# Chaos-Ray-Tracing-Vladislav/course-assignment-DanielHalachev

Measured on AMD Instinct MI355X. Metric: Mpixels/s at 1920x1080 depth 8; HBM GB/s vs roofline, higher is better.
Workload: dtype f32; 1 GPU; HW14 Optimizations02-like BVH scene: room + seeded torus knot + reflective and refractive spheres, four lights, 207954 triangles, 1920x1080, depth 8, 8x8 tiles dealt round-robin over 1 GPU(s); scene=hw14, width=1920, height=1080, max_depth=8, parallelism=tiles8x8-roundrobin-1, tuning=defaults

## Files before the change

course-assignment-danielhalachev_amd/csrc/crt_abi.hip:

```cpp
#include "crt_internal.h"

namespace {


__global__ void unpack_kernel(const float *packed, uint32_t n_parts, uint64_t part_stride, float *frame, uint32_t width,
                              uint32_t height, uint32_t tiles_x, uint32_t n_tiles) {
    const uint64_t gid = (uint64_t)blockIdx.x * blockDim.x + threadIdx.x;
    if (gid >= (uint64_t)n_tiles * 64) return;
    const uint32_t tile = (uint32_t)(gid >> 6), sub = (uint32_t)(gid & 63);
    const uint32_t px = (tile % tiles_x) * TILE + (sub & 7u), py = (tile / tiles_x) * TILE + (sub >> 3);
    if (px >= width || py >= height) return;
    const uint32_t part = tile % n_parts, local = tile / n_parts;
    const float *src = packed + (uint64_t)part * part_stride + ((uint64_t)local * 64 + sub) * 3;
    float *dst = frame + ((uint64_t)py * width + px) * 3;
    dst[0] = src[0]; dst[1] = src[1]; dst[2] = src[2];
}

__global__ void unpack_items_kernel(const float *packed, const WorkItem *items, uint32_t n_items, float *frame, uint32_t width,
                                    uint32_t height, uint32_t tiles_x) {
    const uint64_t gid = (uint64_t)blockIdx.x * blockDim.x + threadIdx.x;
    if (gid >= (uint64_t)n_items * 64) return;
    const WorkItem wi = items[gid >> 6];
    const uint32_t sub = (uint32_t)(gid & 63);
    const uint32_t px = (wi.tile % tiles_x) * TILE + (sub & 7u), py = (wi.tile / tiles_x) * TILE + (sub >> 3);
// ... 147 lines not shown
    const uint32_t n = crt_packed_tile_count(ctx, first, stride);
    crt_rect key{first, stride, 0u, 0u};
    bool same = ctx->cached_is_partition && ctx->cached_rects.size() == 1 && memcmp(ctx->cached_rects.data(), &key, sizeof(key)) == 0;
    if (!same) {
        std::vector<WorkItem> items(n);
        uint64_t pixels = 0;
        for (uint32_t j = 0; j < n; j++) {
            const uint32_t t = first + j * stride;
            const uint32_t tx = t % ctx->tiles_x, ty = t / ctx->tiles_x;
            const uint32_t w = (tx + 1) * TILE <= ctx->width ? TILE : ctx->width - tx * TILE;
            const uint32_t h = (ty + 1) * TILE <= ctx->height ? TILE : ctx->height - ty * TILE;
            pixels += (uint64_t)w * h;
            items[j] = WorkItem{t, j, ~0ull};
        }
        rc = ensure_items(ctx, n ? n : 1);
        if (rc) return rc;
        if (n) CRT_HIP_CHECK(ctx, hipMemcpy(ctx->d_items, items.data(), n * sizeof(WorkItem), hipMemcpyHostToDevice));
        ctx->cached_rects.assign(1, key);
        ctx->cached_is_partition = true;
        ctx->cached_n_items = n;
        ctx->cached_pixels = pixels;
    }
    rc = launch_render(ctx, o, n, d_packed, 1, (hipStream_t)stream);
    if (rc) return rc;
    if (o->collect_counters) {
        CRT_HIP_CHECK(ctx, hipStreamSynchronize((hipStream_t)stream));
        return fetch_counters(ctx, o, ctx->cached_pixels);
    }
    ctx->stats.pixels = ctx->cached_pixels;
    ctx->stats.counters_valid = 0;
    return CRT_OK;
}

extern "C" int crt_unpack_tiles_device(crt_ctx *ctx, const float *d_packed_all, uint32_t n_parts, uint64_t part_stride_floats,
                                       float *d_frame, void *stream) {
    if (!ctx || !d_packed_all || !d_frame || n_parts == 0) return CRT_ERR_INVALID;
    CRT_HIP_CHECK(ctx, hipSetDevice(ctx->device));
    const uint32_t n_tiles = ctx->tiles_x * ctx->tiles_y;
    const uint64_t tiles_per_part = ((uint64_t)n_tiles + n_parts - 1) / n_parts;
    if (part_stride_floats < tiles_per_part * 64 * 3) {
        ctx->error = "crt_unpack_tiles_device: part_stride_floats is smaller than one part's tiles (ceil(tiles / n_parts) * 192 floats)";
        return CRT_ERR_INVALID;
    }
    const uint64_t threads = (uint64_t)n_tiles * 64;
    hipLaunchKernelGGL(unpack_kernel, dim3((uint32_t)((threads + 255) / 256)), dim3(256), 0, (hipStream_t)stream, d_packed_all,
                       n_parts, part_stride_floats, d_frame, ctx->width, ctx->height, ctx->tiles_x, n_tiles);
    CRT_HIP_CHECK(ctx, hipGetLastError());
    return CRT_OK;
}

extern "C" int crt_quantize_device(crt_ctx *ctx, const float *d_rgb, uint64_t n_values, uint8_t *d_out, void *stream) {
    if (!ctx || !d_rgb || !d_out) return CRT_ERR_INVALID;
    CRT_HIP_CHECK(ctx, hipSetDevice(ctx->device));
    if (n_values == 0) return CRT_OK;
    hipLaunchKernelGGL(quantize_kernel, dim3((uint32_t)((n_values + 255) / 256)), dim3(256), 0, (hipStream_t)stream, d_rgb,
                       n_values, d_out);
    CRT_HIP_CHECK(ctx, hipGetLastError());
    return CRT_OK;
}

extern "C" int crt_read_quantized(crt_ctx *ctx, uint8_t *out_rgb8) {
    if (!ctx || !out_rgb8) return CRT_ERR_INVALID;
    const uint64_t n = (uint64_t)ctx->width * ctx->height * 3;
    int rc = crt_quantize_device(ctx, ctx->d_frame, n, ctx->d_quant, ctx->stream);
    if (rc) return rc;
    CRT_HIP_CHECK(ctx, hipMemcpyAsync(out_rgb8, ctx->d_quant, n, hipMemcpyDeviceToHost, ctx->stream));
    CRT_HIP_CHECK(ctx, hipStreamSynchronize(ctx->stream));
    return CRT_OK;
}

extern "C" int crt_kernel_elapsed_ms(crt_ctx *ctx, double *ms) {
    if (!ctx || !ms) return CRT_ERR_INVALID;
    CRT_HIP_CHECK(ctx, hipSetDevice(ctx->device));
    if (ctx->launches == 0) { ctx->error = "no render kernel has been launched"; return CRT_ERR_INVALID; }
    const int slot = (int)((ctx->launches - 1) % crt_ctx::EV_RING);
    CRT_HIP_CHECK(ctx, hipEventSynchronize(ctx->ev4[slot]));
    float f = 0;
    CRT_HIP_CHECK(ctx, hipEventElapsedTime(&f, ctx->ev0[slot], ctx->ev4[slot]));
    *ms = f;
    ctx->stats.kernel_ms = f;
    return CRT_OK;
}

extern "C" int crt_kernel_times_ms(crt_ctx *ctx, double *out_phase_ms, uint32_t max_count, uint32_t *count) {
    if (!ctx || !count) return CRT_ERR_INVALID;
    CRT_HIP_CHECK(ctx, hipSetDevice(ctx->device));
    uint64_t n = ctx->launches < (uint64_t)crt_ctx::EV_RING ? ctx->launches : (uint64_t)crt_ctx::EV_RING;
    if (n > max_count) n = max_count;
    for (uint64_t i = 0; i < n; i++) {
        const int slot = (int)((ctx->launches - n + i) % crt_ctx::EV_RING);
        CRT_HIP_CHECK(ctx, hipEventSynchronize(ctx->ev4[slot]));
        float t = 0, a = 0, b = 0, c = 0, e = 0;
        CRT_HIP_CHECK(ctx, hipEventElapsedTime(&t, ctx->ev0[slot], ctx->ev4[slot]));
        CRT_HIP_CHECK(ctx, hipEventElapsedTime(&a, ctx->ev0[slot], ctx->ev1[slot]));
        CRT_HIP_CHECK(ctx, hipEventElapsedTime(&b, ctx->ev_s0[slot], ctx->ev_s1[slot]));
        hipEvent_t e2 = ctx->ev2[slot];
        if (ctx->slot_ev2_is_s1[slot]) {
            CRT_HIP_CHECK(ctx, hipEventElapsedTime(&c, ctx->ev1[slot], ctx->ev_s1[slot]));
            e2 = c < 0.0f ? ctx->ev1[slot] : ctx->ev_s1[slot];
        }
        CRT_HIP_CHECK(ctx, hipEventElapsedTime(&c, ctx->ev1[slot], e2));
        CRT_HIP_CHECK(ctx, hipEventElapsedTime(&e, e2, ctx->ev3[slot]));
        if (out_phase_ms) {
            out_phase_ms[5 * i] = t; out_phase_ms[5 * i + 1] = a; out_phase_ms[5 * i + 2] = b;
            out_phase_ms[5 * i + 3] = c; out_phase_ms[5 * i + 4] = e;
        }
    }
    *count = (uint32_t)n;
    note_overflow(ctx);
    return CRT_OK;
}

extern "C" int crt_get_kernel_counters(crt_ctx *ctx, uint64_t closest[9], uint64_t shadow[9]) {
    if (!ctx || !closest || !shadow) return CRT_ERR_INVALID;
    for (int k = 0; k < C_PUBLIC; k++) { closest[k] = ctx->level_counters[k]; shadow[k] = ctx->shadow0_counters[k]; }
    return CRT_OK;
}

extern "C" int crt_get_executed_counters(crt_ctx *ctx, uint64_t out[4]) {
    if (!ctx || !out) return CRT_ERR_INVALID;
    out[0] = ctx->exec_counters[0] + ctx->exec_counters[2];
    out[1] = ctx->exec_counters[1] + ctx->exec_counters[3];
    out[2] = ctx->exec_counters[2];
    out[3] = ctx->exec_counters[3];
    return CRT_OK;
}

extern "C" int crt_get_executed_plan_tests(crt_ctx *ctx, uint64_t out[2]) {
    if (!ctx || !out) return CRT_ERR_INVALID;
    out[0] = ctx->exec_counters[4] + ctx->exec_counters[5];
    out[1] = ctx->exec_counters[5];
    return CRT_OK;
}

extern "C" int crt_debug_stream_counts(crt_ctx *ctx, uint32_t *out, uint32_t max_words) {
    if (!ctx || !out) return CRT_ERR_INVALID;
    CRT_HIP_CHECK(ctx, hipSetDevice(ctx->device));
    CRT_HIP_CHECK(ctx, hipDeviceSynchronize());
    const uint32_t n = max_words < (uint32_t)SC_ALLOC_WORDS ? max_words : (uint32_t)SC_ALLOC_WORDS;
    CRT_HIP_CHECK(ctx, hipMemcpy(out, ctx->d_scounts, n * sizeof(uint32_t), hipMemcpyDeviceToHost));
    return CRT_OK;
}

extern "C" int crt_describe_kernels(const crt_ctx *ctx, char *out, size_t size) {
    if (!ctx || !out || size == 0) return CRT_ERR_INVALID;
    const SceneArgs &A = ctx->scene;
    std::string d;
    if (ctx->mode == crt_ctx::MODE_LANES) d = "all=render_lanes<false>";
    else {
        const bool heavy = ctx->step_budget && A.nested_boxes && (A.top_fast || A.plan_seq);
        const bool lean = heavy && ctx->lean_ok && (A.plan_ok || A.plan_wide);
        const bool wide = lean && !A.plan_ok;
        const bool bvh = A.bvh_ok && ctx->tuning.bvh;
        if (bvh && ctx->tuning.level_queue) d = "level0=bvh_trace_level0<0>;shadow0=bvh_trace_shadow<0u, 0>;levels=bvh_trace_queue<0>";
        else if (bvh) d = "level0=bvh_trace_shade;shadow0=bvh_trace_shadow<0u, 0>;levels=bvh_trace_shade";
        else d = std::string("level0=") + (!lean ? "stream_trace_shade<false>" : wide ? "stream_trace_shade_plan_wide" : "stream_trace_shade_plan");
        if (!bvh) d += std::string(";shadow0=") + (!lean ? "stream_trace_shadow<false>" : wide ? "stream_trace_shadow_plan_wide<0u>" : "stream_trace_shadow_plan<0u>");
        if (!bvh) d += std::string(";levels=") + (!heavy ? "stream_trace_shade<false>" : "heavy_trace_closest");
    }
    d += std::string(";filter=") + (A.bvh_ok ? ctx->bvh_stats : "none (" + ctx->bvh_note + ")");
    snprintf(out, size, "%s", d.c_str());
    return CRT_OK;
}

extern "C" int crt_get_stats(crt_ctx *ctx, crt_stats *out) {
    if (!ctx || !out) return CRT_ERR_INVALID;
    *out = ctx->stats;
    return CRT_OK;
}

extern "C" int crt_synchronize(crt_ctx *ctx) {
    if (!ctx) return CRT_ERR_INVALID;
    CRT_HIP_CHECK(ctx, hipSetDevice(ctx->device));
    CRT_HIP_CHECK(ctx, hipDeviceSynchronize());
    note_overflow(ctx);
    return CRT_OK;
}
```

course-assignment-danielhalachev_amd/csrc/crt_internal.h:

```cpp
#pragma once

#include <hip/hip_runtime.h>

#include <algorithm>
#include <cfloat>
#include <cmath>
#include <cstdio>
#include <cstdlib>
#include <chrono>
#include <cstring>
#include <new>
#include <condition_variable>
#include <mutex>
#include <string>
#include <thread>
#include <vector>

#include "../../include/crt_hip.h"
#include "crt_bvh.h"
#include "kernel_common.h"

#define CRT_INTERNAL __attribute__((visibility("hidden")))

constexpr uint64_t QUERY_LAUNCH_RAYS = 1ull << 27;
constexpr uint64_t QUERY_HOST_RAYS = 1ull << 22;
constexpr uint64_t SHOOT_PASS_RAYS = 1ull << 22;

struct crt_ctx {
    int device = 0;
    std::string error;
    hipStream_t stream = nullptr;
    static constexpr int EV_RING = 64;
    hipEvent_t ev0[EV_RING] = {}, ev1[EV_RING] = {}, ev2[EV_RING] = {}, ev3[EV_RING] = {}, ev4[EV_RING] = {};
    hipEvent_t ev_fork[EV_RING] = {}, ev_s0[EV_RING] = {}, ev_s1[EV_RING] = {}, ev_s2[EV_RING] = {};
    bool slot_ev2_is_s1[EV_RING] = {};
    uint64_t launches = 0;
    uint32_t width = 0, height = 0, tiles_x = 0, tiles_y = 0;
    SceneArgs scene{};
    FrameArgs frame{};
    SceneArgs *d_scene = nullptr;
    FrameArgs *d_frame_ring = nullptr, *h_frame_ring = nullptr;
    const FrameArgs *h_frame_ring_dev = nullptr;
    std::vector<void *> allocs;
    float *d_frame = nullptr;
    uint8_t *d_quant = nullptr;
    WorkItem *d_items = nullptr;
    size_t items_cap = 0;
    std::vector<crt_rect> cached_rects;
    bool cached_is_partition = false;
    uint32_t cached_n_items = 0;
    uint64_t cached_pixels = 0;
    uint32_t *d_sync = nullptr;
    uint64_t level_counters[C_N] = {}, shadow0_counters[C_N] = {};
    enum Mode { MODE_STREAM, MODE_LANES } mode = MODE_STREAM;
    float4 *d_rayq[2] = {nullptr, nullptr};
    float4 *d_shadowq = nullptr;
    uint8_t *d_occluded = nullptr;
    float *d_kfac = nullptr;
    float4 *d_nodes = nullptr;
    uint32_t *d_scounts = nullptr;
    unsigned long long *d_exec = nullptr;
    unsigned long long exec_counters[6] = {0, 0, 0, 0, 0, 0};
    uint32_t *d_fallback_total = nullptr;
    uint32_t *d_heavy = nullptr;
    uint32_t *d_sheavy = nullptr;
    float4 *d_hits = nullptr;
    float4 *d_hits_all = nullptr;
    unsigned long long *d_lq = nullptr;
    uint32_t *d_lq_words = nullptr;
    uint32_t *d_bvh_spill = nullptr;
    uint32_t bvh_stack_built = 0;
    size_t bvh_spill_words() const { return bvh_stack_built > BVH_LDS_STACK ? (size_t)grid_blocks * BLOCK * (bvh_stack_built - BVH_LDS_STACK) : 0u; }
    hipStream_t side = nullptr;
    hipStream_t early = nullptr;
    hipEvent_t ev_reset[EV_RING] = {}, ev_queue[EV_RING] = {};
    static constexpr uint32_t H_SLOT_WORDS = 512;
    uint32_t *h_ring = nullptr;
    uint64_t next_count_harvest = 0;
    uint32_t slot_items[EV_RING] = {};
    std::vector<uint32_t> last_counts;
    uint32_t last_counts_items = 0;
    uint32_t fallbacks_seen = 0;
    double node_mult = 4.0, ray_mult = 2.0, shadow_extra = 1.0;
    uint32_t sizing_seen_fallbacks = 0;
    uint64_t queue_bytes = 0;
    uint64_t regrows = 0;
    uint32_t last_counts_cfg = 0;
    uint32_t slot_cfg[64] = {};
    hipEvent_t ev_call0 = nullptr, ev_call1 = nullptr;
    bool pending = false;
    crt_options pending_options{};
    uint32_t heavy_cap = 0;
    uint32_t step_budget = 384;
    bool lean_ok = true;
    uint64_t stream_items = 0;
    uint64_t overflows = 0;
    uint32_t n_lights = 0;
    crt_tuning tuning{};
    std::string bvh_note;
    std::string bvh_stats;
    unsigned long long *d_counters = nullptr;
    float *d_frames = nullptr;
    size_t frames_floats = 0;
    uint32_t grid_blocks = 0;
    crt_stats stats{};
    int num_cus = 0;
    struct crt_query_state *query = nullptr;
    uint64_t query_host_rays = QUERY_HOST_RAYS, query_launch_rays = QUERY_LAUNCH_RAYS, shoot_pass_rays = SHOOT_PASS_RAYS;
};

static constexpr uint32_t HEAVY_BLOCKS = 4096;
static constexpr uint32_t REFILL_BUNDLE = 16;

extern CRT_INTERNAL std::string g_create_error;

#define CRT_HIP_CHECK(ctx, expr)                                                                    \
    do {                                                                                            \
        hipError_t e_ = (expr);                                                                     \
        if (e_ != hipSuccess) {                                                                     \
            (ctx)->error = std::string(#expr) + ": " + hipGetErrorString(e_);                       \
            return CRT_ERR_HIP;                                                                     \
        }                                                                                           \
    } while (0)

template <typename T>
static int upload(crt_ctx *ctx, const T *src, size_t count, const T **dst) {
    void *p = nullptr;
    size_t bytes = (count ? count : 1) * sizeof(T);
    CRT_HIP_CHECK(ctx, hipMalloc(&p, bytes));
    ctx->allocs.push_back(p);
    if (count) CRT_HIP_CHECK(ctx, hipMemcpy(p, src, count * sizeof(T), hipMemcpyHostToDevice));
    *dst = (const T *)p;
    return CRT_OK;
}

CRT_INTERNAL int check_options(crt_ctx *ctx, const crt_options *o);
CRT_INTERNAL int ensure_items(crt_ctx *ctx, size_t n);
CRT_INTERNAL int launch_render(crt_ctx *ctx, const crt_options *o, uint32_t n_items, float *d_out, uint32_t packed, hipStream_t stream);
CRT_INTERNAL void note_overflow(crt_ctx *ctx);
CRT_INTERNAL int fetch_counters(crt_ctx *ctx, const crt_options *o, uint64_t pixels);
CRT_INTERNAL void query_destroy(crt_ctx *ctx);
CRT_INTERNAL uint64_t coverage_items(uint32_t width, uint32_t height, const crt_rect *rects, uint32_t n_rects, std::vector<WorkItem> &items);
CRT_INTERNAL void launch_unpack_items(const float *packed, const WorkItem *items, uint32_t n_items, float *frame, uint32_t width, uint32_t height,
                                      uint32_t tiles_x, hipStream_t stream);
```

course-assignment-danielhalachev_amd/csrc/crt_launch.hip:

```cpp
#include "crt_internal.h"
#include "glibc_powf.h"

namespace {

#include "kernel_lane.h"
#include "kernel_stream.h"
#include "kernel_heavy.h"
#include "kernel_plan.h"
#include "kernel_bvh.h"

}

int check_options(crt_ctx *ctx, const crt_options *o) {
    if (!o) { ctx->error = "options is NULL"; return CRT_ERR_INVALID; }
    if (o->use_gi && o->collect_counters == 2) { ctx->error = "collect_counters == 2 belongs to the ray-stream kernels; the GI mode renders with render_lanes"; return CRT_ERR_INVALID; }
    if (o->use_gi && (o->gi_sample_size > 64u || o->rays_per_pixel > 65536u)) { ctx->error = "gi_sample_size > 64 or rays_per_pixel > 65536"; return CRT_ERR_INVALID; }
    if (o->max_depth > 4096) { ctx->error = "max_depth too large"; return CRT_ERR_INVALID; }
    return CRT_OK;
}

int ensure_items(crt_ctx *ctx, size_t n) {
    if (n <= ctx->items_cap) return CRT_OK;
    CRT_HIP_CHECK(ctx, hipDeviceSynchronize());
    if (ctx->d_items) (void)hipFree(ctx->d_items);
// ... 134 lines not shown
        CRT_HIP_CHECK(ctx, hipMalloc((void **)&ctx->d_hits, (size_t)ctx->heavy_cap * sizeof(float4)));
        CRT_HIP_CHECK(ctx, hipMalloc((void **)&ctx->d_hits_all, (size_t)std::max<uint64_t>(ray_cap, px) * sizeof(float4)));
        if (ctx->scene.bvh_ok && ctx->tuning.bvh && ctx->tuning.level_queue) {
            CRT_HIP_CHECK(ctx, hipMalloc((void **)&ctx->d_lq, node_cap * 8 * sizeof(unsigned long long)));
            CRT_HIP_CHECK(ctx, hipMemset(ctx->d_lq, 0, node_cap * 8 * sizeof(unsigned long long)));
        }
        A.s_ray_cap = (uint32_t)ray_cap; A.s_shadow_cap = (uint32_t)shadow_cap; A.s_node_cap = (uint32_t)node_cap;
        ctx->stream_items = n_items;
        ctx->queue_bytes = ray_cap * 64 + shadow_cap * 37 + node_cap * 32 + (size_t)ctx->heavy_cap * 24 + std::max<uint64_t>(ray_cap, px) * 16 + (ctx->d_lq ? node_cap * 64 : 0);
    }
    A.s_rayq[0] = ctx->d_rayq[0]; A.s_rayq[1] = ctx->d_rayq[1];
    A.s_shadowq = ctx->d_shadowq; A.s_occluded = ctx->d_occluded; A.s_kfac = ctx->d_kfac; A.s_nodes = ctx->d_nodes;
    A.s_heavy = ctx->d_heavy; A.s_sheavy = ctx->d_sheavy; A.s_hits = ctx->d_hits; A.s_hits_all = ctx->d_hits_all; A.s_heavy_cap = ctx->heavy_cap;
    A.s_lq = ctx->d_lq; A.s_lq_cap = ctx->d_lq ? (ctx->tuning.ray_cap ? std::min(A.s_ray_cap, A.s_node_cap) : A.s_node_cap) : 0u;
    return CRT_OK;
}

static uint32_t level0_samples_of(const crt_options *o) { return o->use_gi && o->rays_per_pixel > 1u ? o->rays_per_pixel : 1u; }
static bool gi_fits_stream(const crt_options *o, uint32_t n_items) {
    return (uint64_t)n_items * 64u * level0_samples_of(o) * 2u < (1ull << 31) && o->gi_sample_size <= 64u;
}
static uint32_t frame_config_of(const crt_options *o) {
    return (o->use_gi ? 0x80000000u : 0u) | ((o->use_gi ? o->gi_sample_size & 0x7Fu : 0u) << 24) | (o->max_depth & 0xFFFFFFu);
}

static int g_debug_sync = 0;
template <typename K, typename... Args>
static void launch(K kernel, uint32_t blocks, hipStream_t stream, Args... args) {
    static int serial = 0;
    if (g_debug_sync) { fprintf(stderr, "[launch %d] kernel %p blocks %u ...", serial, (void *)kernel, blocks); fflush(stderr); }
    hipLaunchKernelGGL(kernel, dim3(blocks), dim3(BLOCK), 0, stream, args...);
    if (g_debug_sync) { hipError_t e = hipDeviceSynchronize(); fprintf(stderr, " done (%s)\n", hipGetErrorString(e)); fflush(stderr); serial++; }
}
template <typename K, typename... Args>
static void launch_lds(K kernel, uint32_t blocks, uint32_t lds_bytes, hipStream_t stream, Args... args) {
    hipLaunchKernelGGL(kernel, dim3(blocks), dim3(BLOCK), lds_bytes, stream, args...);
}

struct FramePlan {
    int slot;
    uint32_t n_items, vitems;
    uint32_t lane_blocks;
    bool gi, count, exec_count;
    bool heavy, lean, wide;
    bool bvh;
    bool queue;
    uint32_t widest;
    uint32_t level_budget;
    const uint32_t *prev;
    bool last_resort;
    bool one_stream;
};

static void launch_frame_reset(crt_ctx *ctx, const FramePlan &P, hipStream_t stream, bool stream_pass, uint32_t shadow_preset, uint32_t split_preset) {
    hipLaunchKernelGGL(stream_frame_reset, dim3(1), dim3(256), 0, stream, stream_pass ? ctx->d_scounts : (uint32_t *)nullptr,
                       stream_pass && P.queue ? ctx->d_lq_words : (uint32_t *)nullptr, stream_pass && P.exec_count ? ctx->d_exec : (unsigned long long *)nullptr,
                       shadow_preset, split_preset, ctx->d_sync, (uint32_t *)(ctx->d_frame_ring + P.slot), (const uint32_t *)(ctx->h_frame_ring_dev + P.slot));
}

static int launch_stream_levels(crt_ctx *ctx, const crt_options *o, FramePlan &P, KernelArgs &A, hipStream_t stream) {
    const uint32_t fixed_slots = ctx->frame.fixed0 ? (uint32_t)P.vitems * 64u * ctx->n_lights : 0u;
    const bool split_known = P.queue && ctx->frame.fixed0;
    launch_frame_reset(ctx, P, stream, true, fixed_slots, split_known ? fixed_slots : 0u);
    const uint32_t side_per_cu = ctx->tuning.side_blocks;
    A.exec_count = P.exec_count ? 1u : 0u;
    A.exec_counters = ctx->d_exec;
    A.exec_plan = ctx->d_exec + 4;
    A.bundle = REFILL_BUNDLE;
    A.wave_prio = 3u;
    A.force_whole = 0u;
    const uint32_t plds = ctx->scene.plan_list_words * BLOCK * (uint32_t)sizeof(uint32_t);
    A.chunk = ctx->tuning.fetch_chunk >> 16;
    KernelArgs S = A;
    S.wave_prio = 0u;
    S.chunk = ctx->tuning.fetch_chunk & 0xFFFFu;
    S.counters = ctx->d_counters + C_N;
    S.exec_counters = ctx->d_exec + 2;
    S.exec_plan = ctx->d_exec + 5;
    {
        const uint64_t lanes = (uint64_t)ctx->num_cus * (side_per_cu ? side_per_cu : 8u) * BLOCK;
        const uint64_t est = (uint64_t)P.vitems * 64u * (ctx->n_lights ? ctx->n_lights : 1u) * 130u / (lanes ? lanes : 1u);
        uint32_t budget = est > ctx->tuning.shadow_budget ? ctx->tuning.shadow_budget : (uint32_t)est;
        if (budget < ctx->step_budget) budget = std::min(ctx->step_budget, ctx->tuning.shadow_budget);
        S.step_budget = P.heavy ? budget : 0u;
    }
    const uint32_t *prev = ctx->last_counts_items == P.vitems && ctx->last_counts_cfg == frame_config_of(o) && !ctx->last_counts[SC_OVERFLOW] ? ctx->last_counts.data() : nullptr;
    const uint32_t level_budget = (P.wide || P.gi) ? std::min<uint32_t>(ctx->step_budget * 4u, 1u << 20) : ctx->step_budget;
    P.prev = prev; P.level_budget = level_budget;
    const uint64_t est0 = (uint64_t)P.vitems * 64u * 70u / ((uint64_t)P.lane_blocks * BLOCK);
    uint32_t budget0 = est0 >= level_budget ? level_budget : (est0 < 64u ? 64u : (uint32_t)est0);
    if (ctx->tuning.level0_budget) budget0 = ctx->tuning.level0_budget;
    const bool early_queue = P.queue && side_per_cu && !(ctx->tuning.level_queue & 512u) && !g_debug_sync;
    P.one_stream = early_queue && P.bvh && split_known && !(ctx->tuning.level_queue & 4096u);
    auto launch_queue = [&](hipStream_t where) {
        KernelArgs Q = A;
        const uint32_t qblocks = std::min(P.lane_blocks, (uint32_t)ctx->num_cus * std::max(1u, ctx->tuning.level_queue & 15u));
        Q.force_whole = (P.widest > 70000u || (ctx->tuning.level_queue & 256u)) ? 1u : 0u;
        Q.bundle = ctx->tuning.level0_budget ? ctx->tuning.level0_budget - 1u : 15u;
        if (P.exec_count) launch(bvh_trace_queue<BVH_TALLY>, qblocks, where, Q);
        else if (ctx->tuning.bvh == 2) launch(bvh_trace_queue<BVH_CHECKED>, qblocks, where, Q);
        else launch(bvh_trace_queue<BVH_PLAIN>, qblocks, where, Q);
    };
    for (uint32_t g = 0; g <= o->max_depth; g++) {
        A.step_budget = P.heavy ? (g == 0 ? budget0 : level_budget) : 0u;
        uint32_t level_blocks = P.lane_blocks;
        if (g >= 1 && P.lean && prev) {
            const uint32_t was = prev[SC_COUNT + g];
            const uint32_t want = was < ctx->frame.heavy_level_threshold ? 64u : std::max<uint32_t>((uint32_t)ctx->num_cus, (was + was / 2u + BLOCK - 1) / BLOCK);
            level_blocks = std::min(P.lane_blocks, want);
        }
        if (P.queue && g == 0) {
            if (early_queue && o->max_depth >= 1) {
                CRT_HIP_CHECK(ctx, hipEventRecord(ctx->ev_reset[P.slot], stream));
                CRT_HIP_CHECK(ctx, hipStreamWaitEvent(ctx->early, ctx->ev_reset[P.slot], 0));
                launch_queue(ctx->early);
                if (ctx->tuning.level_queue & 4096u) {
                    CRT_HIP_CHECK(ctx, hipEventRecord(ctx->ev_queue[P.slot], ctx->early));
                    CRT_HIP_CHECK(ctx, hipStreamWaitEvent(stream, ctx->ev_queue[P.slot], 0));
                }
            }
            if (P.exec_count) launch(bvh_trace_level0<BVH_TALLY>, P.lane_blocks, stream, A);
            else if (ctx->tuning.bvh == 2) launch(bvh_trace_level0<BVH_CHECKED>, P.lane_blocks, stream, A);
            else launch(bvh_trace_level0<BVH_PLAIN>, P.lane_blocks, stream, A);
        }
        else if (P.bvh && P.gi) {
            launch(bvh_trace_shade_gi, P.lane_blocks, stream, A, g);
            launch(stream_shade_all<true>, P.lane_blocks, stream, A, g);
        }
        else if (P.bvh) launch(P.exec_count ? bvh_trace_shade_tally : ctx->tuning.bvh == 2 ? bvh_trace_shade_checked : bvh_trace_shade, g == 0 ? P.lane_blocks : level_blocks, stream, A, g);
        else if (P.count) { if (P.gi) launch(stream_trace_shade<true, true>, P.lane_blocks, stream, A, g); else launch(stream_trace_shade<true>, P.lane_blocks, stream, A, g); }
        else if (P.lean && P.gi) {
            launch_lds(P.wide ? stream_trace_plan_wide_gi : stream_trace_plan_gi, level_blocks, plds, stream, A, g);
            launch(stream_shade_all<true>, level_blocks, stream, A, g);
        }
        else if (P.wide) launch_lds(stream_trace_shade_plan_wide, level_blocks, plds, stream, A, g);
        else if (P.lean) launch_lds(stream_trace_shade_plan, level_blocks, plds, stream, A, g);
        else if (P.gi) launch(stream_trace_shade<false, true>, P.lane_blocks, stream, A, g);
        else launch(stream_trace_shade<false>, P.lane_blocks, stream, A, g);
        if (P.heavy && !P.bvh) {
            launch(P.gi ? heavy_trace_closest_gi : P.exec_count ? heavy_trace_closest_tally : heavy_trace_closest, HEAVY_BLOCKS, stream, A, g);
            if (P.gi) launch(stream_shade_evicted<false, true>, 256u, stream, A, g);
            else launch(stream_shade_evicted<false>, 256u, stream, A, g);
        }
        if (g == 0) {
            if (!split_known) hipLaunchKernelGGL(stream_mark_split, dim3(1), dim3(64), 0, stream, A, (uint32_t)SC_SHADOW_SPLIT, (uint32_t)SC_SHADOW);
            hipStream_t where = side_per_cu && !P.one_stream ? ctx->side : stream;
            if (side_per_cu && !P.one_stream) {
                CRT_HIP_CHECK(ctx, hipEventRecord(ctx->ev_fork[P.slot], stream));
                CRT_HIP_CHECK(ctx, hipStreamWaitEvent(ctx->side, ctx->ev_fork[P.slot], 0));
            }
            if (P.one_stream && o->max_depth == 0) CRT_HIP_CHECK(ctx, hipEventRecord(ctx->ev1[P.slot], stream));
            CRT_HIP_CHECK(ctx, hipEventRecord(ctx->ev_s0[P.slot], where));
            const uint32_t blocks0 = side_per_cu ? std::min(ctx->grid_blocks, (uint32_t)ctx->num_cus * side_per_cu) : ctx->grid_blocks;
            if (P.bvh) {
                if (P.exec_count) launch(bvh_trace_shadow<0, BVH_TALLY>, blocks0, where, S);
                else if (ctx->tuning.bvh == 2) launch(bvh_trace_shadow<0, BVH_CHECKED>, blocks0, where, S);
                else launch(bvh_trace_shadow<0, BVH_PLAIN>, blocks0, where, S);
            }
            else if (P.count) launch(stream_trace_shadow<true>, blocks0, where, S, 0u);
            else if (P.wide) launch(stream_trace_shadow_plan_wide<0>, blocks0, where, S);
            else if (P.lean) launch(stream_trace_shadow_plan<0>, blocks0, where, S);
            else launch(stream_trace_shadow<false>, blocks0, where, S, 0u);
            if (P.heavy && !P.bvh) hipLaunchKernelGGL(stream_mark_split, dim3(1), dim3(64), 0, where, S, (uint32_t)SC_SHEAVY_SPLIT, (uint32_t)SC_SHEAVY);
            CRT_HIP_CHECK(ctx, hipEventRecord(ctx->ev_s1[P.slot], where));
            if (P.heavy && !P.bvh) launch(P.exec_count ? heavy_trace_shadow_tally : heavy_trace_shadow, HEAVY_BLOCKS, where, S, 0u);
            if (!P.one_stream) CRT_HIP_CHECK(ctx, hipEventRecord(ctx->ev_s2[P.slot], where));
        }
        if (P.queue) {
            if (early_queue && o->max_depth >= 1) {
                CRT_HIP_CHECK(ctx, hipStreamWaitEvent(ctx->early, P.one_stream ? ctx->ev_s0[P.slot] : ctx->ev_fork[P.slot], 0));
                launch_queue(ctx->early);
                if (P.one_stream) CRT_HIP_CHECK(ctx, hipEventRecord(ctx->ev1[P.slot], ctx->early));
                CRT_HIP_CHECK(ctx, hipEventRecord(ctx->ev_queue[P.slot], ctx->early));
                CRT_HIP_CHECK(ctx, hipStreamWaitEvent(stream, ctx->ev_queue[P.slot], 0));
            }
            else if (o->max_depth >= 1) launch_queue(stream);
            break;
        }
    }
    return CRT_OK;
}

static int launch_stream_tail(crt_ctx *ctx, FramePlan &P, KernelArgs &A, hipStream_t stream) {
    const uint32_t side_per_cu = ctx->tuning.side_blocks;
    const uint32_t *prev = P.prev;
    const uint32_t level_budget = P.level_budget;
    CRT_HIP_CHECK(ctx, hipGetLastError());
    if (!P.one_stream) CRT_HIP_CHECK(ctx, hipEventRecord(ctx->ev1[P.slot], stream));
    if (side_per_cu && !P.one_stream) CRT_HIP_CHECK(ctx, hipStreamWaitEvent(stream, ctx->ev_s1[P.slot], 0));
    KernelArgs S1 = A;
    S1.wave_prio = 0u;
    S1.counters = ctx->d_counters + 2 * C_N;
    {
        const uint64_t rays1 = prev && prev[SC_SHADOW] >= prev[SC_SHADOW_SPLIT] ? prev[SC_SHADOW] - prev[SC_SHADOW_SPLIT] : (uint64_t)P.vitems * 16u;
        const uint64_t est1 = rays1 * 130u / ((uint64_t)P.lane_blocks * BLOCK);
        const uint32_t cap1 = std::max(level_budget, ctx->tuning.shadow_budget);
        S1.step_budget = P.heavy ? (est1 >= cap1 ? cap1 : (est1 < 64u ? 64u : (uint32_t)est1)) : 0u;
    }
    if (P.queue) {}
    else if (P.bvh) {
        if (P.exec_count) launch(bvh_trace_shadow<1, BVH_TALLY>, P.lane_blocks, stream, S1);
        else if (ctx->tuning.bvh == 2) launch(bvh_trace_shadow<1, BVH_CHECKED>, P.lane_blocks, stream, S1);
        else launch(bvh_trace_shadow<1, BVH_PLAIN>, P.lane_blocks, stream, S1);
    }
    else if (P.count) launch(stream_trace_shadow<true>, P.lane_blocks, stream, S1, 1u);
    else if (P.wide) launch(stream_trace_shadow_plan_wide<1>, P.lane_blocks, stream, S1);
    else if (P.lean) launch(stream_trace_shadow_plan<1>, P.lane_blocks, stream, S1);
    else launch(stream_trace_shadow<false>, P.lane_blocks, stream, S1, 1u);
    if (side_per_cu && !P.one_stream) CRT_HIP_CHECK(ctx, hipStreamWaitEvent(stream, ctx->ev_s2[P.slot], 0));
    if (P.heavy && !P.bvh) launch(P.exec_count ? heavy_trace_shadow_tally : heavy_trace_shadow, HEAVY_BLOCKS, stream, S1, 1u);
    CRT_HIP_CHECK(ctx, hipGetLastError());
    if (!P.one_stream) CRT_HIP_CHECK(ctx, hipEventRecord(ctx->ev2[P.slot], stream));
    A.counters = ctx->d_counters + 2 * C_N;
    if (P.count) launch(stream_resolve<true>, P.lane_blocks, stream, A);
    else launch(stream_resolve<false>, P.lane_blocks, stream, A);
    A.only_if_overflow = 1;
    const uint32_t fallback_blocks = std::max(1u, std::min(ctx->grid_blocks, (P.n_items * 64u + BLOCK - 1) / BLOCK));
    if (!P.last_resort) {}
    else if (P.gi && P.count) launch(render_lanes<true, true>, fallback_blocks, stream, A);
    else if (P.gi) launch(render_lanes<false, true>, fallback_blocks, stream, A);
    else if (P.count) launch(render_lanes<true>, fallback_blocks, stream, A);
    else launch(render_lanes<false>, fallback_blocks, stream, A);
    CRT_HIP_CHECK(ctx, hipGetLastError());
    return CRT_OK;
}

static int launch_lanes_pass(crt_ctx *ctx, FramePlan &P, KernelArgs &A, hipStream_t stream) {
    launch_frame_reset(ctx, P, stream, false, 0u, 0u);
    CRT_HIP_CHECK(ctx, hipEventRecord(ctx->ev1[P.slot], stream));
    A.counters = ctx->d_counters + C_N;
    if (P.gi && P.count) launch(render_lanes<true, true>, P.lane_blocks, stream, A);
    else if (P.gi) launch(render_lanes<false, true>, P.lane_blocks, stream, A);
    else if (P.count) launch(render_lanes<true>, P.lane_blocks, stream, A);
    else launch(render_lanes<false>, P.lane_blocks, stream, A);
    CRT_HIP_CHECK(ctx, hipGetLastError());
    for (hipEvent_t e : {ctx->ev_s0[P.slot], ctx->ev_s1[P.slot], ctx->ev_s2[P.slot], ctx->ev2[P.slot]}) CRT_HIP_CHECK(ctx, hipEventRecord(e, stream));
    return CRT_OK;
}

static int launch_frame(crt_ctx *ctx, const crt_options *o, uint32_t n_items, float *d_out, uint32_t packed, hipStream_t stream, bool last_resort) {
    const bool gi = o->use_gi != 0;
    int rc = ensure_frames(ctx, o->max_depth, gi);
    if (rc) return rc;
    const SceneArgs &SC = ctx->scene;
    FrameArgs &F = ctx->frame;
    F.use_gi = gi ? 1u : 0u;
    F.gi_samples = o->gi_sample_size;
    F.rays_per_pixel = o->rays_per_pixel;
    F.monte_carlo_bias = o->monte_carlo_bias;
    F.gi_seed = o->gi_seed;
    const uint32_t samples = level0_samples_of(o);
    const bool stream_mode = ctx->mode == crt_ctx::MODE_STREAM && (!gi || gi_fits_stream(o, n_items));
    const uint32_t vitems = stream_mode ? n_items * samples : n_items;
    F.level0_samples = stream_mode ? samples : 1u;
    if (stream_mode && o->max_depth + 1 > (uint32_t)MAX_GENERATIONS) {
        ctx->error = "max_depth too large for the ray-stream pass";
        return CRT_ERR_INVALID;
    }
    F.max_depth = o->max_depth;
    F.shadow_bias = o->shadow_bias;
    F.reflection_bias = o->reflection_bias;
    F.refraction_bias = o->refraction_bias;
    F.items = ctx->d_items;
    F.n_items = n_items;
    F.pixel_counter = ctx->d_sync + 0;
    F.out = d_out;
    F.packed = packed;
    F.s_counts = ctx->d_scounts;
    F.fallback_total = ctx->d_fallback_total;
    F.s_lq_words = ctx->d_lq_words;
    F.lq_epoch = (uint32_t)(ctx->launches & 0x7FFFFFFFull) + 1u;
    F.bvh_spill = ctx->d_bvh_spill;
    F.bvh_spill_side = ctx->d_bvh_spill ? ctx->d_bvh_spill + ctx->bvh_spill_words() : nullptr;
    F.bvh_spill_queue = ctx->d_bvh_spill ? ctx->d_bvh_spill + 2u * ctx->bvh_spill_words() : nullptr;
    F.bvh_spill_words = ctx->d_bvh_spill ? ctx->bvh_spill_words() : 0u;
    const bool count = o->collect_counters == 1;
    const bool exec_count = o->collect_counters == 2;
    if (count) CRT_HIP_CHECK(ctx, hipMemsetAsync(ctx->d_counters, 0, 3 * C_N * sizeof(unsigned long long), stream));
    harvest_counts(ctx);
    const int slot = (int)(ctx->launches % crt_ctx::EV_RING);
    if (ctx->launches >= (uint64_t)crt_ctx::EV_RING) {
        CRT_HIP_CHECK(ctx, hipEventSynchronize(ctx->ev4[slot]));
        harvest_counts(ctx);
    }
    ctx->slot_items[slot] = 0;
    const uint32_t lane_need = (vitems * 64u + BLOCK - 1) / BLOCK;
    const uint32_t lane_blocks = std::max(1u, lane_need < ctx->grid_blocks ? lane_need : ctx->grid_blocks);
    CRT_HIP_CHECK(ctx, hipEventRecord(ctx->ev0[slot], stream));
    if (n_items == 0) {
        for (hipEvent_t e : {ctx->ev1[slot], ctx->ev_s0[slot], ctx->ev_s1[slot], ctx->ev_s2[slot], ctx->ev2[slot], ctx->ev3[slot], ctx->ev4[slot]})
            CRT_HIP_CHECK(ctx, hipEventRecord(e, stream));
        ctx->slot_ev2_is_s1[slot] = false;
        ctx->launches++;
        return CRT_OK;
    }
    const bool heavy = stream_mode && ctx->step_budget && SC.nested_boxes && (SC.top_fast || SC.plan_seq) && !count;
    const bool lean = heavy && ctx->lean_ok && (SC.plan_ok || SC.plan_wide);
    const bool wide = lean && !SC.plan_ok;
    const bool bvh = stream_mode && SC.bvh_ok && ctx->tuning.bvh && !count && !(gi && (exec_count || ctx->tuning.bvh == 2));
    uint32_t widest = 0;
    if (ctx->last_counts_items == vitems && ctx->last_counts_cfg == frame_config_of(o))
        for (uint32_t g = 1; g <= o->max_depth && g < (uint32_t)MAX_GENERATIONS; g++) widest = std::max(widest, ctx->last_counts[SC_COUNT + g]);
    const bool queue = bvh && !gi && ctx->tuning.level_queue && last_resort && widest <= 250000u;
    g_debug_sync = ctx->tuning.bvh == 3 ? 1 : 0;
    if (g_debug_sync) fprintf(stderr, "[frame] bvh_trace_shade %p tally %p checked %p shadow0 %p shadow1 %p heavy_closest %p shade_evicted %p resolve %p heavy_shadow %p\n",
                              (void *)bvh_trace_shade, (void *)bvh_trace_shade_tally, (void *)bvh_trace_shade_checked, (void *)bvh_trace_shadow<0, BVH_PLAIN>,
                              (void *)bvh_trace_shadow<1, BVH_PLAIN>, (void *)heavy_trace_closest, (void *)stream_shade_evicted<false>, (void *)stream_resolve<false>, (void *)heavy_trace_shadow);
// ... 77 lines not shown
```

course-assignment-danielhalachev_amd/csrc/kernel_bvh.h:

```cpp
#pragma once

#include "crt_bvh.h"
#include "kernel_common.h"
#include "kernel_stream.h"
#include "kernel_walk.h"

struct BvhStack { uint32_t *lds; uint32_t *spill; uint32_t stride; size_t room; };
__device__ __forceinline__ void bvh_push(const BvhStack &S, uint32_t &sp, const uint32_t v) {
    if (sp < BVH_LDS_STACK) S.lds[sp * BLOCK] = v;
    else S.spill[(size_t)(sp - BVH_LDS_STACK) * S.stride] = v;
    sp++;
}
__device__ __forceinline__ uint32_t bvh_pop(const BvhStack &S, uint32_t &sp) {
    sp--;
    return sp < BVH_LDS_STACK ? S.lds[sp * BLOCK] : S.spill[(size_t)(sp - BVH_LDS_STACK) * S.stride];
}
enum : int { BVH_SPILL_LEVELS = 0,
             BVH_SPILL_SIDE = 1,
             BVH_SPILL_QUEUE = 2 };
__device__ __forceinline__ BvhStack bvh_stack_of(const KernelArgs &A, uint32_t *stack_lds, const int region) {
    BvhStack S;
    S.lds = stack_lds + threadIdx.x;
    S.stride = gridDim.x * BLOCK;
    const size_t column = (size_t)blockIdx.x * BLOCK + threadIdx.x;
// ... 453 lines not shown
    const BvhStack stack = bvh_stack_of(A, stack_lds, BVH_SPILL_QUEUE);
    const unsigned long long below = (1ull << lane) - 1ull;
    uint32_t nbox = 0, ntri = 0;
    Ray R;
    R.ox = R.oy = R.oz = R.dx = R.dy = R.dz = R.ix = R.iy = R.iz = 0; R.parmask = 0;
    BvhWalk W;
    bvh_walk_begin(W, INFINITY);
    int state = BVH_FETCH;
    uint32_t r = 0, gen = 1, spins = 0, idle_polls = 0, early_polls = 0;
    uint32_t sh_first = 0, sh_stride = 0, sh_li = 0, sh_slot = 0;
    bool sh_walking = false;
    float light_dist = 0;
    const uint32_t n_lights = A.s->n_lights;
    for (;;) {
        if (++spins > (1u << 20)) { A.f->s_counts[SC_GUARD] = 1; A.f->s_counts[SC_OVERFLOW] = 1; __hip_atomic_store(ovf_p, 1u, __ATOMIC_RELAXED, __HIP_MEMORY_SCOPE_AGENT); break; }
        const unsigned long long fin = __ballot(state == BVH_FINISHED), idle = __ballot(state == BVH_FETCH);
        const bool walking = __ballot(state == BVH_WALK || state == BVH_MISS_CHECK || state == BVH_SHADOWS) != 0;
        const uint32_t n_walk = (uint32_t)__popcll(__ballot(state == BVH_WALK || state == BVH_MISS_CHECK || state == BVH_SHADOWS));
        if ((uint32_t)__popcll(fin) >= BVH_BATCH || !walking || (fin && n_walk <= 8u) || ((fin | idle) && (spins & A.bundle) == 0u)) {
            if (state == BVH_FINISHED) {
                if (MODE == BVH_TALLY && gen < 10u) {
                    uint32_t *dg = A.f->s_counts + SC_BVH_DIAG + 48 + 3 * gen;
                    atomicMax(dg + 0, W.steps); atomicAdd(dg + 1, W.steps); atomicAdd(dg + 2, 1u);
                }
                if (W.give_up) { A.f->s_counts[SC_GUARD] = 1; A.f->s_counts[SC_OVERFLOW] = 1; __hip_atomic_store(ovf_p, 1u, __ATOMIC_RELAXED, __HIP_MEMORY_SCOPE_AGENT); }
                bool diffuse = false;
                float keep[6];
                uint32_t keep_index = NONE;
                shade_and_emit<false, false, true>(A, gen, r, count0, count0, R, W.have, W.best, W.btri, W.bmesh, nullptr, lane, &diffuse, &sh_first, &sh_stride,
                                                   A.force_whole ? nullptr : keep, &keep_index);
                state = (diffuse && n_lights) ? BVH_SHADOWS : BVH_FETCH;
                sh_li = 0; sh_walking = false;
                if (keep_index != NONE) {
                    r = keep_index; gen = gen + 1u;
                    R.ox = keep[0]; R.oy = keep[1]; R.oz = keep[2]; R.dx = keep[3]; R.dy = keep[4]; R.dz = keep[5];
                    normalize3(R.dx, R.dy, R.dz);
                    ray_prepare(R);
                    bvh_walk_begin(W, INFINITY);
                    if (bvh_ray_setup(A, R, W.B)) state = BVH_WALK;
                    else { W.give_up = true; state = BVH_FINISHED; }
                }
            }
            uint32_t t = 0, h = 0;
            if (lane == 0) {
                if (fin) atomicAdd(A.f->s_lq_words + LQ_DONE, (uint32_t)__popcll(fin));
                t = __hip_atomic_load(tail_p, __ATOMIC_RELAXED, __HIP_MEMORY_SCOPE_AGENT);
                h = __hip_atomic_load(head_p, __ATOMIC_RELAXED, __HIP_MEMORY_SCOPE_AGENT);
            }
            t = __builtin_amdgcn_readfirstlane(t); h = __builtin_amdgcn_readfirstlane(h);
            const unsigned long long want = __ballot(state == BVH_FETCH);
            const uint32_t n_want = (uint32_t)__popcll(want), avail = t > h ? t - h : 0u;
            const uint32_t take = n_want < avail ? n_want : avail;
            if (take) {
                uint32_t base = 0;
                if (lane == 0) base = atomicAdd(A.f->s_lq_words + LQ_HEAD, take);
                base = __builtin_amdgcn_readfirstlane(base);
                const uint32_t rank = (uint32_t)__popcll(want & below);
                if (state == BVH_FETCH && rank < take) { r = base + rank; state = BVH_WAIT; }
                idle_polls = 0;
            } else if (n_want || __ballot(state == BVH_WAIT)) {
                uint32_t d = 0, t2 = 0, ovf = 0, l0 = 0;
                if (lane == 0) {
                    l0 = __hip_atomic_load(l0_p, __ATOMIC_RELAXED, __HIP_MEMORY_SCOPE_AGENT);
                    asm volatile("s_waitcnt vmcnt(0)" ::: "memory");
                    d = __hip_atomic_load(done_p, __ATOMIC_RELAXED, __HIP_MEMORY_SCOPE_AGENT);
                    asm volatile("s_waitcnt vmcnt(0)" ::: "memory");
                    t2 = __hip_atomic_load(tail_p, __ATOMIC_RELAXED, __HIP_MEMORY_SCOPE_AGENT);
                    ovf = __hip_atomic_load(ovf_p, __ATOMIC_RELAXED, __HIP_MEMORY_SCOPE_AGENT);
                }
                d = __builtin_amdgcn_readfirstlane(d); t2 = __builtin_amdgcn_readfirstlane(t2); ovf = __builtin_amdgcn_readfirstlane(ovf);
                l0 = __builtin_amdgcn_readfirstlane(l0);
                if (!l0 && early_polls < 160u) { early_polls++; idle_polls = 0; }
                if ((ovf || (l0 && d == t2)) && (state == BVH_FETCH || ovf || (state == BVH_WAIT && r >= t2))) state = BVH_OUT;
                if (!__ballot(state != BVH_FETCH && state != BVH_OUT) && ++idle_polls >= 4u) state = BVH_OUT;
            }
        }
        if (state == BVH_WAIT) {
            uint32_t level = 0;
            const int what = lq_load_ray(A, r, R.ox, R.oy, R.oz, R.dx, R.dy, R.dz, level);
            if (what == LQ_TAKEN) state = BVH_FETCH;
            if (what == LQ_RAY) {
                gen = level;
                normalize3(R.dx, R.dy, R.dz);
                ray_prepare(R);
                bvh_walk_begin(W, INFINITY);
                if (bvh_ray_setup(A, R, W.B)) state = BVH_WALK;
                else { W.give_up = true; state = BVH_FINISHED; }
            }
        }
        if (!__ballot(state != BVH_OUT)) break;
        if (state == BVH_SHADOWS && !sh_walking) {
            sh_slot = sh_first + sh_li * sh_stride;
            const float4 q0 = A.f->s_shadowq[2 * (size_t)sh_slot], q1 = A.f->s_shadowq[2 * (size_t)sh_slot + 1];
            if (q1.w == 0.0f) {
                A.f->s_occluded[sh_slot] = 0;
                if (++sh_li == n_lights) state = BVH_FETCH;
            } else {
                R.ox = q0.x; R.oy = q0.y; R.oz = q0.z;
                R.dx = q1.x; R.dy = q1.y; R.dz = q1.z;
                ray_prepare(R);
                light_dist = q0.w;
                bvh_walk_begin(W, light_dist * (1.0f + 0x1p-16f));
                if (bvh_ray_setup(A, R, W.B)) sh_walking = true;
                else { A.f->s_counts[SC_GUARD] = 1; A.f->s_counts[SC_OVERFLOW] = 1; A.f->s_occluded[sh_slot] = 0; if (++sh_li == n_lights) state = BVH_FETCH; }
            }
        }
        if (!__ballot(state == BVH_WALK || state == BVH_MISS_CHECK || state == BVH_FINISHED || state == BVH_SHADOWS)) {
            __builtin_amdgcn_s_sleep(127);
            if (idle_polls >= 1u) __builtin_amdgcn_s_sleep(127);
            if (idle_polls >= 2u) { __builtin_amdgcn_s_sleep(127); __builtin_amdgcn_s_sleep(127); }
        }
        {
            const bool sh_lane = state == BVH_SHADOWS;
            bool stepping = state == BVH_WALK || (sh_lane && sh_walking);
            for (int it = 0; it < BVH_STEPS_QUEUE; ++it)
                if (stepping && !bvh_step<2, MODE>(A, R, false, light_dist, false, W, stack, nbox, ntri, sh_lane)) {
                    stepping = false;
                    if (sh_lane) {
                        if (W.give_up) { A.f->s_counts[SC_GUARD] = 1; A.f->s_counts[SC_OVERFLOW] = 1; }
                        A.f->s_occluded[sh_slot] = W.have ? 1 : 0;
                        sh_walking = false;
                        if (++sh_li == n_lights) state = BVH_FETCH;
                    } else if (W.have || W.give_up) state = BVH_FINISHED;
                    else { W.cur = 0; W.sp = 0; W.cache_mesh = NONE; W.cache_k2 = NONE; bvh_line_setup(A, R, W.B); state = BVH_MISS_CHECK; }
                }
        }
        if (state == BVH_MISS_CHECK) {
            for (int it = 0; it < BVH_STEPS_QUEUE; ++it)
                if (state == BVH_MISS_CHECK && !bvh_miss_step<MODE>(A, R, false, W, stack, nbox, ntri)) state = BVH_FINISHED;
        }
    }
    exec_counters_flush(A, nbox, ntri, lane);
}
template <int MODE>
__global__ __launch_bounds__(BLOCK) void bvh_trace_queue(const KernelArgs A) {
    __shared__ uint32_t stack_lds[BVH_LDS_STACK * BLOCK];
    bvh_queue_levels<MODE>(A, stack_lds);
}

template <int MODE, bool CHUNKED>
__device__ __forceinline__ void bvh_shadow_rays(const KernelArgs &A, const uint32_t first, const uint32_t total, uint32_t *cursor, uint32_t *stack_lds) {
    const uint32_t lane = threadIdx.x & 63u;
    if (A.f->s_counts[SC_OVERFLOW]) return;
    const BvhStack stack = bvh_stack_of(A, stack_lds, BVH_SPILL_SIDE);
    const bool every_mesh = A.f->use_gi != 0;
    const uint32_t fixed_end = level0_fixed_slots(A);
    uint32_t nbox = 0, ntri = 0;
    Ray R;
    R.ox = R.oy = R.oz = R.dx = R.dy = R.dz = R.ix = R.iy = R.iz = 0; R.parmask = 0;
    BvhWalk W;
    bvh_walk_begin(W, INFINITY);
    float light_dist = 0;
    int state = BVH_FETCH;
    uint32_t r = 0, spins = 0;
    WaveChunk chunk{0u, 0u};
    for (;;) {
        if (MODE == BVH_CHECKED && ++spins > (1u << 22)) { bvh_at<MODE>(A, spins, 0u, 15); break; }
        const uint32_t n_free = (uint32_t)__popcll(__ballot(state == BVH_FETCH || state == BVH_FINISHED));
        if (n_free >= BVH_BATCH || (n_free && !__ballot(state == BVH_WALK))) {
            if (state == BVH_FINISHED) {
                if (MODE == BVH_TALLY) {
                    uint32_t *dg = A.f->s_counts + SC_BVH_DIAG + 40;
                    if (atomicMax(dg + 0, W.steps) < W.steps) dg[1] = r;
                    atomicAdd(dg + 2, W.steps >> 4);
                    if (W.steps >= 1024u) atomicAdd(dg + 3, 1u);
                }
                if (W.give_up) { A.f->s_counts[SC_GUARD] = 1; A.f->s_counts[SC_OVERFLOW] = 1; }
                A.f->s_occluded[r] = W.have ? 1 : 0;
                state = BVH_FETCH;
            }
            uint32_t claimed = 0;
            if (CHUNKED) claimed = wave_fetch_chunked(cursor, lane, state == BVH_FETCH, chunk, A.chunk, total);
            if (state == BVH_FETCH) {
                r = CHUNKED ? claimed : wave_fetch(cursor, lane);
                if (r >= total) state = BVH_OUT;
                else {
                    r += first;
                    float kfac;
                    bool used;
                    if (r < fixed_end) used = level0_shadow_ray(A, r, R, light_dist, kfac);
                    else {
                        const float4 q0 = A.f->s_shadowq[2 * (size_t)r], q1 = A.f->s_shadowq[2 * (size_t)r + 1];
                        used = __float_as_uint(q0.w) != SHADOW_SLOT_UNUSED;
                        R.ox = q0.x; R.oy = q0.y; R.oz = q0.z;
                        R.dx = q1.x; R.dy = q1.y; R.dz = q1.z;
                        ray_prepare(R);
                        light_dist = q0.w; kfac = q1.w;
                    }
                    if (!used) {}
                    else if (kfac == 0.0f) A.f->s_occluded[r] = 0;
                    else {
                        bvh_walk_begin(W, light_dist * (1.0f + 0x1p-16f));
                        if (bvh_ray_setup(A, R, W.B)) state = BVH_WALK;
                        else { W.give_up = true; state = BVH_FINISHED; }
                    }
                }
            }
        }
        if (!__ballot(state != BVH_OUT)) break;
        if (state == BVH_WALK) {
            for (int it = 0; it < BVH_STEPS; ++it)
                if (state == BVH_WALK && !bvh_step<1, MODE>(A, R, false, light_dist, every_mesh, W, stack, nbox, ntri)) state = BVH_FINISHED;
        }
    }
    exec_counters_flush(A, nbox, ntri, lane);
}
template <uint32_t pass, int MODE>
__global__ __launch_bounds__(BLOCK) void bvh_trace_shadow(const KernelArgs A) {
    __shared__ uint32_t stack_lds[BVH_LDS_STACK * BLOCK];
    const uint32_t split = A.f->s_counts[SC_SHADOW_SPLIT];
    bvh_shadow_rays<MODE, pass == 0>(A, pass == 0 ? 0u : split, pass == 0 ? split : A.f->s_counts[SC_SHADOW] - split,
                          A.f->s_counts + (pass == 0 ? SC_SHADOW_FETCH : SC_SHADOW_FETCH2), stack_lds);
}
```

Measured before the change: 860.4 Mpixels/s.

## Trace level-0 shadow rays per pixel, looping over lights within one lane

Adds a per-pixel shadow kernel for level 0. Each lane claims a pixel and walks the BVH once per light, accumulating the lit contribution and writing the shaded result directly, instead of each lane claiming a single shadow-ray slot. The kernel is used when the BVH path is on, the level-0 slots are fixed and GI is off. The fetch chunk is divided by the light count, and the walk refills lanes every few steps. This cuts per-ray slot fetches, slot reads and the separate occlusion writes, but adds serial work per lane and may lower coherence between lanes.

```diff
diff --git a/course-assignment-danielhalachev_amd/csrc/crt_abi.hip b/course-assignment-danielhalachev_amd/csrc/crt_abi.hip
--- a/course-assignment-danielhalachev_amd/csrc/crt_abi.hip
+++ b/course-assignment-danielhalachev_amd/csrc/crt_abi.hip
@@ -323,8 +323,9 @@
         const bool lean = heavy && ctx->lean_ok && (A.plan_ok || A.plan_wide);
         const bool wide = lean && !A.plan_ok;
         const bool bvh = A.bvh_ok && ctx->tuning.bvh;
-        if (bvh && ctx->tuning.level_queue) d = "level0=bvh_trace_level0<0>;shadow0=bvh_trace_shadow<0u, 0>;levels=bvh_trace_queue<0>";
-        else if (bvh) d = "level0=bvh_trace_shade;shadow0=bvh_trace_shadow<0u, 0>;levels=bvh_trace_shade";
+        const char *shadow0 = ctx->shadow0_by_slot ? ";shadow0=bvh_trace_shadow<0u, 0, false>" : ";shadow0=bvh_trace_shadow<0u, 0, true>";
+        if (bvh && ctx->tuning.level_queue) d = std::string("level0=bvh_trace_level0<0>") + shadow0 + ";levels=bvh_trace_queue<0>";
+        else if (bvh) d = std::string("level0=bvh_trace_shade") + shadow0 + ";levels=bvh_trace_shade";
         else d = std::string("level0=") + (!lean ? "stream_trace_shade<false>" : wide ? "stream_trace_shade_plan_wide" : "stream_trace_shade_plan");
         if (!bvh) d += std::string(";shadow0=") + (!lean ? "stream_trace_shadow<false>" : wide ? "stream_trace_shadow_plan_wide<0u>" : "stream_trace_shadow_plan<0u>");
         if (!bvh) d += std::string(";levels=") + (!heavy ? "stream_trace_shade<false>" : "heavy_trace_closest");
diff --git a/course-assignment-danielhalachev_amd/csrc/crt_internal.h b/course-assignment-danielhalachev_amd/csrc/crt_internal.h
--- a/course-assignment-danielhalachev_amd/csrc/crt_internal.h
+++ b/course-assignment-danielhalachev_amd/csrc/crt_internal.h
@@ -34,6 +34,7 @@
     hipEvent_t ev0[EV_RING] = {}, ev1[EV_RING] = {}, ev2[EV_RING] = {}, ev3[EV_RING] = {}, ev4[EV_RING] = {};
     hipEvent_t ev_fork[EV_RING] = {}, ev_s0[EV_RING] = {}, ev_s1[EV_RING] = {}, ev_s2[EV_RING] = {};
     bool slot_ev2_is_s1[EV_RING] = {};
+    bool shadow0_by_slot = false;
     uint64_t launches = 0;
     uint32_t width = 0, height = 0, tiles_x = 0, tiles_y = 0;
     SceneArgs scene{};
diff --git a/course-assignment-danielhalachev_amd/csrc/crt_launch.hip b/course-assignment-danielhalachev_amd/csrc/crt_launch.hip
--- a/course-assignment-danielhalachev_amd/csrc/crt_launch.hip
+++ b/course-assignment-danielhalachev_amd/csrc/crt_launch.hip
@@ -310,7 +310,15 @@
             if (P.one_stream && o->max_depth == 0) CRT_HIP_CHECK(ctx, hipEventRecord(ctx->ev1[P.slot], stream));
             CRT_HIP_CHECK(ctx, hipEventRecord(ctx->ev_s0[P.slot], where));
             const uint32_t blocks0 = side_per_cu ? std::min(ctx->grid_blocks, (uint32_t)ctx->num_cus * side_per_cu) : ctx->grid_blocks;
-            if (P.bvh) {
+            const bool by_pixel = P.bvh && ctx->frame.fixed0 && !P.gi;
+            if (P.bvh) ctx->shadow0_by_slot = !by_pixel;
+            if (by_pixel) {
+                S.chunk = std::max(64u, (S.chunk / std::max(1u, ctx->n_lights)) & ~63u);
+                if (P.exec_count) launch(bvh_trace_shadow<0, BVH_TALLY, true>, blocks0, where, S);
+                else if (ctx->tuning.bvh == 2) launch(bvh_trace_shadow<0, BVH_CHECKED, true>, blocks0, where, S);
+                else launch(bvh_trace_shadow<0, BVH_PLAIN, true>, blocks0, where, S);
+            }
+            else if (P.bvh) {
                 if (P.exec_count) launch(bvh_trace_shadow<0, BVH_TALLY>, blocks0, where, S);
                 else if (ctx->tuning.bvh == 2) launch(bvh_trace_shadow<0, BVH_CHECKED>, blocks0, where, S);
                 else launch(bvh_trace_shadow<0, BVH_PLAIN>, blocks0, where, S);
diff --git a/course-assignment-danielhalachev_amd/csrc/kernel_bvh.h b/course-assignment-danielhalachev_amd/csrc/kernel_bvh.h
--- a/course-assignment-danielhalachev_amd/csrc/kernel_bvh.h
+++ b/course-assignment-danielhalachev_amd/csrc/kernel_bvh.h
@@ -629,7 +629,7 @@
     bvh_walk_begin(W, INFINITY);
     float light_dist = 0;
     int state = BVH_FETCH;
-    uint32_t r = 0, spins = 0;
+    uint32_t r = 0, spins = 0, issued = 0;
     WaveChunk chunk{0u, 0u};
     for (;;) {
         if (MODE == BVH_CHECKED && ++spins > (1u << 22)) { bvh_at<MODE>(A, spins, 0u, 15); break; }
@@ -641,6 +641,7 @@
                     if (atomicMax(dg + 0, W.steps) < W.steps) dg[1] = r;
                     atomicAdd(dg + 2, W.steps >> 4);
                     if (W.steps >= 1024u) atomicAdd(dg + 3, 1u);
+                    atomicAdd(dg + 4, W.steps); atomicAdd(dg + 5, 1u);
                 }
                 if (W.give_up) { A.f->s_counts[SC_GUARD] = 1; A.f->s_counts[SC_OVERFLOW] = 1; }
                 A.f->s_occluded[r] = W.have ? 1 : 0;
@@ -675,17 +676,99 @@
             }
         }
         if (!__ballot(state != BVH_OUT)) break;
+        if (MODE == BVH_TALLY && __ballot(state == BVH_WALK)) issued += (uint32_t)BVH_STEPS;
         if (state == BVH_WALK) {
             for (int it = 0; it < BVH_STEPS; ++it)
                 if (state == BVH_WALK && !bvh_step<1, MODE>(A, R, false, light_dist, every_mesh, W, stack, nbox, ntri)) state = BVH_FINISHED;
         }
     }
+    if (MODE == BVH_TALLY && lane == 0) atomicAdd(A.f->s_counts + SC_BVH_DIAG + 46, issued);
     exec_counters_flush(A, nbox, ntri, lane);
 }
-template <uint32_t pass, int MODE>
+
+constexpr int BVH_PIXEL_RESTART = 8;
+static_assert(BVH_STEPS % BVH_PIXEL_RESTART == 0, "a turn is a whole number of restart intervals");
+template <int MODE>
+__device__ __forceinline__ void bvh_shadow_pixels(const KernelArgs &A, uint32_t *stack_lds) {
+    const uint32_t lane = threadIdx.x & 63u;
+    if (A.f->s_counts[SC_OVERFLOW]) return;
+    const uint32_t n_lights = A.s->n_lights;
+    if (!n_lights) return;
+    const uint32_t total = stream_level_count(A, 0);
+    uint32_t *cursor = A.f->s_counts + SC_SHADOW_FETCH;
+    const BvhStack stack = bvh_stack_of(A, stack_lds, BVH_SPILL_SIDE);
+    uint32_t nbox = 0, ntri = 0;
+    Ray R;
+    R.ox = R.oy = R.oz = R.dx = R.dy = R.dz = R.ix = R.iy = R.iz = 0; R.parmask = 0;
+    BvhWalk W;
+    bvh_walk_begin(W, INFINITY);
+    float light_dist = 0, kfac = 0, ax = 0, ay = 0, az = 0, albx = 0, alby = 0, albz = 0;
+    int state = BVH_FETCH;
+    uint32_t r = 0, li = 0, spins = 0, issued = 0;
+    WaveChunk chunk{0u, 0u};
+    auto light_ended = [&](const bool blocked) {
+        if (!blocked) { ax += kfac * albx; ay += kfac * alby; az += kfac * albz; }
+        if (++li == n_lights) {
+            A.f->s_nodes[2 * (size_t)r] = make_float4(ax, ay, az, __uint_as_float(TN_CONST));
+            state = BVH_FETCH;
+        } else state = BVH_SHADOWS;
+    };
+    for (;;) {
+        if (MODE == BVH_CHECKED && ++spins > (1u << 22)) { bvh_at<MODE>(A, spins, 0u, 15); break; }
+        const uint32_t n_free = (uint32_t)__popcll(__ballot(state == BVH_FETCH));
+        if (n_free >= BVH_BATCH || (n_free && !__ballot(state == BVH_WALK || state == BVH_SHADOWS))) {
+            const uint32_t claimed = wave_fetch_chunked(cursor, lane, state == BVH_FETCH, chunk, A.chunk, total);
+            if (state == BVH_FETCH) {
+                r = claimed;
+                if (r >= total) state = BVH_OUT;
+                else {
+                    const float4 p = A.f->s_shadowq[2 * (size_t)r], n0 = A.f->s_nodes[2 * (size_t)r];
+                    if (__float_as_uint(p.w) != SHADOW_SLOT_UNUSED) {
+                        const uint32_t kind = __float_as_uint(n0.w);
+                        if ((kind & (TN_KIND_MASK | TN_GI)) != TN_DIFFUSE) bvh_at<MODE>(A, kind, 0u, 13);
+                        else { albx = n0.x; alby = n0.y; albz = n0.z; ax = ay = az = 0; li = 0; state = BVH_SHADOWS; }
+                    }
+                }
+            }
+        }
+        if (!__ballot(state != BVH_OUT)) break;
+        for (int part = 0; part < BVH_STEPS / BVH_PIXEL_RESTART; ++part) {
+            if (state == BVH_SHADOWS) {
+                const float4 p = A.f->s_shadowq[2 * (size_t)r], n = A.f->s_shadowq[2 * (size_t)r + 1];
+                light_setup(A, li, p.x, p.y, p.z, n.x, n.y, n.z, R, light_dist, kfac);
+                if (kfac == 0.0f) light_ended(false);
+                else {
+                    bvh_walk_begin(W, light_dist * (1.0f + 0x1p-16f));
+                    if (bvh_ray_setup(A, R, W.B)) state = BVH_WALK;
+                    else { A.f->s_counts[SC_GUARD] = 1; A.f->s_counts[SC_OVERFLOW] = 1; light_ended(false); }
+                }
+            }
+            if (MODE == BVH_TALLY && __ballot(state == BVH_WALK)) issued += (uint32_t)BVH_PIXEL_RESTART;
+            for (int it = 0; it < BVH_PIXEL_RESTART; ++it)
+                if (state == BVH_WALK && !bvh_step<1, MODE>(A, R, false, light_dist, false, W, stack, nbox, ntri)) {
+                    if (MODE == BVH_TALLY) {
+                        uint32_t *dg = A.f->s_counts + SC_BVH_DIAG + 40;
+                        if (atomicMax(dg + 0, W.steps) < W.steps) dg[1] = r;
+                        atomicAdd(dg + 2, W.steps >> 4);
+                        if (W.steps >= 1024u) atomicAdd(dg + 3, 1u);
+                        atomicAdd(dg + 4, W.steps); atomicAdd(dg + 5, 1u);
+                    }
+                    if (W.give_up) { A.f->s_counts[SC_GUARD] = 1; A.f->s_counts[SC_OVERFLOW] = 1; }
+                    light_ended(W.have);
+                }
+        }
+    }
+    if (MODE == BVH_TALLY && lane == 0) atomicAdd(A.f->s_counts + SC_BVH_DIAG + 46, issued);
+    exec_counters_flush(A, nbox, ntri, lane);
+}
+template <uint32_t pass, int MODE, bool PIXELS = false>
 __global__ __launch_bounds__(BLOCK) void bvh_trace_shadow(const KernelArgs A) {
     __shared__ uint32_t stack_lds[BVH_LDS_STACK * BLOCK];
-    const uint32_t split = A.f->s_counts[SC_SHADOW_SPLIT];
-    bvh_shadow_rays<MODE, pass == 0>(A, pass == 0 ? 0u : split, pass == 0 ? split : A.f->s_counts[SC_SHADOW] - split,
-                          A.f->s_counts + (pass == 0 ? SC_SHADOW_FETCH : SC_SHADOW_FETCH2), stack_lds);
-}
+    static_assert(!PIXELS || pass == 0, "only level 0's slots are fixed ones");
+    if constexpr (PIXELS) bvh_shadow_pixels<MODE>(A, stack_lds);
+    else {
+        const uint32_t split = A.f->s_counts[SC_SHADOW_SPLIT];
+        bvh_shadow_rays<MODE, pass == 0>(A, pass == 0 ? 0u : split, pass == 0 ? split : A.f->s_counts[SC_SHADOW] - split,
+                              A.f->s_counts + (pass == 0 ? SC_SHADOW_FETCH : SC_SHADOW_FETCH2), stack_lds);
+    }
+}
```

Measured after the change: 890.2 Mpixels/s, median of 6. 1.03x the previous value.
